# LuZWCHA/MLIC

Measured on AMD Instinct MI355X. Metric: images/sec (enc+dec) at 1920×1088 MLICPP_L, 1/2/4/8 GPU; bpp/PSNR Δ vs ref, higher is better.
Workload: dtype f32 (dense convs: f32 via split-fp16 MFMA, 3 terms); 1 GPU; config 2: MLICPP_L compress+decompress of 1920x1088 images (full rANS bitstreams, inputs resident in HBM); model=MLICPP_L, global_batch=32, per_gpu_images=32, weights=rate set(s) [1] of synthetic.RATE_LAMBDAS, parallelism=image-sharded x1 (no cross-GPU context), request_streams=4, schedule=each request stream runs its K steps back to back (no per-step join)

## Files before the change

mlic_amd/csrc/conv_x4.hip:

```cpp
#include "common.h"
#include "kernels.h"

#include <cstdio>
#include <type_traits>
#include <utility>
#include <vector>

namespace mlic {

typedef float floatx4 __attribute__((ext_vector_type(4)));
typedef _Float16 half8 __attribute__((ext_vector_type(8)));

namespace {
constexpr int X4T = 512;
constexpr int TR = 8, TC = 32;
constexpr int BN = TR * TC;
constexpr int ROWB = 128;
constexpr int ROWH = 64;

__device__ __forceinline__ int swz(int row) { return (row >> 1) & 7; }

__device__ __forceinline__ void glds16(const void* src, void* lds) {
  __builtin_amdgcn_global_load_lds((const __attribute__((address_space(1))) void*)src,
                                   (__attribute__((address_space(3))) void*)lds, 16, 0, 0);
}

__device__ __forceinline__ void glds16_asm(const void* src, const void* lds) {
  const uint32_t l = __builtin_amdgcn_readfirstlane(
      (uint32_t)reinterpret_cast<uintptr_t>((const __attribute__((address_space(3))) void*)lds));
  asm volatile("s_mov_b32 m0, %1\n\ts_nop 0\n\tglobal_load_lds_dwordx4 %0, off" : : "v"(src), "s"(l) : "m0");
}

__device__ __forceinline__ half8 lds_frag(const char* base, int row, int granule) {
  return *reinterpret_cast<const half8*>(base + row * ROWB + ((granule ^ swz(row)) << 4));
}
}

#ifndef MLIC_X4_ABL_RS
#define MLIC_X4_ABL_RS 0
#endif
#ifndef MLIC_X4_SPREAD
#define MLIC_X4_SPREAD 0
#endif
#ifndef MLIC_X4_STAGGER
#define MLIC_X4_STAGGER 0
#endif
template <int K, int BM, bool RS, bool HI, bool DIR = false, bool HALO = false>
__global__ __launch_bounds__(X4T) void conv_x4_kernel(ConvParams P, const _Float16* __restrict__ act,
                                                      const _Float16* __restrict__ wx, int nchunk, int H, int W,
                                                      int abl, int nsplit) {
  constexpr int KK = K * K;
  constexpr int WAVES_M = BM == 192 ? 4 : (BM == 96 || BM == 224) ? 2 : BM / 64, WAVES_N = 8 / WAVES_M;
  constexpr int WN = BN / WAVES_N;
  constexpr int TM = BM / (16 * WAVES_M), TN = WN / 16;
  constexpr int WR = 16 * TM;
  constexpr int A_BYTES = BM * ROWB, B_BYTES = BN * ROWB;
  constexpr int NAB = RS ? 2 : 3;
  constexpr int HR = TR + K - 1, HC = TC + K - 1, HLINES = HR * HC;
  constexpr int BSLOT = HALO ? HLINES * ROWB : B_BYTES;
  constexpr int B_OFF = NAB * A_BYTES, LDS = NAB * A_BYTES + 2 * BSLOT;
  constexpr int NA = A_BYTES / 1024 / 8;
  constexpr int NB = B_BYTES / 1024 / 8;
  static_assert(NA >= 1 && NB == 4 && LDS <= 160 * 1024, "x4 tile");
  static_assert(!HALO || (RS && !DIR && K > 1), "x4 halo: register-staged K x K only");
  __shared__ __attribute__((aligned(1024))) char sm[LDS];

  const int tid = threadIdx.x, lane = tid & 63, wave = tid >> 6;
  const int wm = wave / WAVES_N, wn = wave % WAVES_N;
  const int pad = K / 2;
  const int npix = P.Ho * P.Wo;
  const int S = K == 1 ? 1 : P.stride;
  const int Hp = (K == 1 ? H : P.H) + 2 * pad, Wp = (K == 1 ? W : P.W) + 2 * pad;
  const int ntx = (W + TC - 1) / TC;
  const int nct = gridDim.x, npt = gridDim.y, nblk = nct * npt;
  const int bid = blockIdx.y * nct + blockIdx.x;
  int logical = bid;
  if (nblk >= 16) {
    const int xcd = bid & 7, q = nblk >> 3, r = nblk & 7;
    logical = (xcd < r ? xcd * (q + 1) : r * (q + 1) + (xcd - r) * q) + (bid >> 3);
  }
  constexpr int XG = 4;
  int ct, pt;
  if (K == 1 && nct >= 2 * XG) {
    const int band = XG * npt, g = logical / band, first = g * XG, r = logical - g * band;
    const int gs = min(XG, nct - first);
    ct = first + r % gs;
    pt = r / gs;
  } else {
    ct = logical % nct;
    pt = logical / nct;
  }
  const int oy0 = (pt / ntx) * TR, ox0 = (pt % ntx) * TC;
  const int b = blockIdx.z % P.B, split = blockIdx.z / P.B;
  const int nsteps = nchunk * KK;
  const int s0 = HALO ? split * nchunk / nsplit * KK : split * nsteps / nsplit;
  const int s1 = HALO ? (split + 1) * nchunk / nsplit * KK : (split + 1) * nsteps / nsplit;
  if (nsplit > 1) P.out += (int64_t)split * P.B * P.out_bs;

  const int64_t plane = (int64_t)Hp * Wp * ROWH;
  const _Float16* bsrc[NB];
#pragma unroll
  for (int i = 0; i < NB; ++i) {
    const int n = (wave * NB + i) * 8 + (lane >> 3);
    const int oy = min(oy0 + n / TC, H - 1), ox = min(ox0 + n % TC, W - 1);
    const int G = (lane & 7) ^ swz(n);
    bsrc[i] = act + (int64_t)b * nchunk * plane + ((int64_t)oy * S * Wp + ox * S) * ROWH + G * 8;
  }
  const _Float16* asrc = wx + ((int64_t)ct * nsteps * BM) * ROWH + (wave * NA) * 512 + lane * 8;

  auto glds_one = [&](int g, int sb, int sa, int abuf) {
    if (g < NB) {
      const int cc = sb / KK, tap = sb - cc * KK;
      const int ky = tap / K, kx = tap - ky * K;
      const int64_t d = cc * plane + ((int64_t)ky * Wp + kx) * ROWH;
      glds16_asm(bsrc[g] + d, sm + B_OFF + (sb & 1) * B_BYTES + (wave * NB + g) * 1024);
    } else {
      const int i = g - NB;
      glds16_asm(asrc + (int64_t)sa * BM * ROWH + i * 512, sm + abuf * A_BYTES + (wave * NA + i) * 1024);
    }
  };
  constexpr int NG = NA + NB;

  floatx4 acc[TM][TN];
#pragma unroll
  for (int i = 0; i < TM; ++i)
#pragma unroll
    for (int j = 0; j < TN; ++j) acc[i][j] = floatx4{0.f, 0.f, 0.f, 0.f};

  const int G = lane >> 4, l16 = lane & 15;
  if constexpr (RS) {
    typedef unsigned int u32x4 __attribute__((ext_vector_type(4)));
    constexpr int NPA = A_BYTES / 1024, NAR = (NPA + 7) / 8;
    constexpr bool SPREAD = MLIC_X4_SPREAD && !DIR && !HALO && !HI;
    const _Float16* asrc_rs = wx + ((int64_t)ct * nsteps * BM) * ROWH + wave * 512 + lane * 8;
    u32x4 rb[(DIR || HALO) ? 1 : NB], ra[NAR];
    constexpr int NPH = (HLINES * 8 + X4T - 1) / X4T;
    static_assert(!HALO || NPH + 1 <= KK, "x4 halo: the next chunk's pieces must land within the chunk");
    u32x4 hb;
    const _Float16* himg = act + (int64_t)b * nchunk * plane;
    auto hsrc = [&](int q) __attribute__((always_inline)) {
      const int id = q * X4T + tid, line = min(id >> 3, HLINES - 1);
      const int hr = line / HC, hc = line - hr * HC;
      const int y = min(oy0 + hr, Hp - 1), x = min(ox0 + hc, Wp - 1);
      return ((int64_t)y * Wp + x) * ROWH + (id & 7) * 8;
    };
    auto hdst = [&](int q, int slot) __attribute__((always_inline)) {
      const int id = q * X4T + tid, line = id >> 3;
      return sm + B_OFF + slot * BSLOT + line * ROWB + (((id & 7) ^ swz(line)) << 4);
    };
    auto hvalid = [&](int q) __attribute__((always_inline)) { return q * X4T + tid < HLINES * 8; };
    float rv[DIR ? 16 : 1];
    const int dn = (wave & 3) * 64 + lane, dch = (wave >> 2) * 16;
    const int dp = min(oy0 * TC + dn, npix - 1);
    uint32_t dmax = 0;
    auto gload = [&](int st) __attribute__((always_inline)) {
      const int cc = st / KK, tap = st - cc * KK;
      const int ky = tap / K, kx = tap - ky * K;
      if constexpr (DIR) {
        const int ch0 = cc * 32 + dch;
        const float* sp = P.seg[0].p;
        int64_t sbs = P.seg[0].bs;
        int c0 = 0, cend = 0;
#pragma unroll
        for (int k = 1; k < MAXSEG; ++k) {
          cend += P.seg[k - 1].C;
          uint64_t pk = (uint64_t)P.seg[k].p, bk = (uint64_t)P.seg[k].bs;
          asm("" : "+s"(pk), "+s"(bk));
          if (k < P.nseg && ch0 >= cend) {
            sp = (const float*)pk;
            sbs = (int64_t)bk;
            c0 = cend;
          }
        }
        typedef const __attribute__((address_space(1))) float gfloat;
        gfloat* src = (gfloat*)(sp + (int64_t)b * sbs + (int64_t)(ch0 - c0) * npix) + dp;
        const int nval = P.Cin - ch0;
        if (nval >= 16) {
#pragma unroll
          for (int j = 0; j < 16; ++j) rv[j] = src[(int64_t)j * npix];
        } else {
#pragma unroll
          for (int j = 0; j < 16; ++j) rv[j] = j < nval ? src[(int64_t)j * npix] : 0.0f;
        }
      } else if constexpr (!HALO) {
        const int64_t d = cc * plane + ((int64_t)ky * Wp + kx) * ROWH;
#pragma unroll
        for (int i = 0; i < NB; ++i) rb[i] = *reinterpret_cast<const u32x4*>(bsrc[i] + d);
      }
#pragma unroll
      for (int i = 0; i < NAR; ++i)
        if (NPA % 8 == 0 || wave + 8 * i < NPA)
          ra[i] = *reinterpret_cast<const u32x4*>(asrc_rs + (int64_t)st * BM * ROWH + i * 8 * 512);
    };
    auto lstore = [&](int st) __attribute__((always_inline)) {
      if constexpr (DIR) {
        typedef float float2v __attribute__((ext_vector_type(2)));
        typedef _Float16 half2v __attribute__((ext_vector_type(2)));
        char* row = sm + B_OFF + (st & 1) * B_BYTES + dn * ROWB;
        const int sw = swz(dn), g0 = dch / 8;
#pragma unroll
        for (int q = 0; q < 2; ++q) {
          half8 h, l;
#pragma unroll
          for (int j = 0; j < 8; j += 2) {
            const float2v v = {rv[8 * q + j], rv[8 * q + j + 1]};
            const half2v hv = __builtin_convertvector(v, half2v);
            const half2v lv = __builtin_convertvector(v - __builtin_convertvector(hv, float2v), half2v);
            h[j] = hv[0];
            h[j + 1] = hv[1];
            l[j] = lv[0];
            l[j + 1] = lv[1];
            dmax = max(dmax, max(__float_as_uint(v[0]) & 0x7fffffffu, __float_as_uint(v[1]) & 0x7fffffffu));
          }
          *reinterpret_cast<half8*>(row + (((g0 + q) ^ sw) << 4)) = h;
          *reinterpret_cast<half8*>(row + (((g0 + q + 4) ^ sw) << 4)) = l;
        }
      } else if constexpr (!HALO) {
#pragma unroll
        for (int i = 0; i < NB; ++i)
          *reinterpret_cast<u32x4*>(sm + B_OFF + (st & 1) * B_BYTES + (wave * NB + i) * 1024 + lane * 16) = rb[i];
      }
#pragma unroll
      for (int i = 0; i < NAR; ++i)
        if (NPA % 8 == 0 || wave + 8 * i < NPA)
          *reinterpret_cast<u32x4*>(sm + (st & 1) * A_BYTES + (wave + 8 * i) * 1024 + lane * 16) = ra[i];
    };
    constexpr int NPC = NB + NAR;
    auto gload_piece = [&](int st, int p) __attribute__((always_inline)) {
      if (p < NB) {
        const int cc = st / KK, tap = st - cc * KK;
        const int ky = tap / K, kx = tap - ky * K;
        const int64_t d = cc * plane + ((int64_t)ky * Wp + kx) * ROWH;
        rb[p] = *reinterpret_cast<const u32x4*>(bsrc[p] + d);
      } else {
        const int i = p - NB;
        if (NPA % 8 == 0 || wave + 8 * i < NPA)
          ra[i] = *reinterpret_cast<const u32x4*>(asrc_rs + (int64_t)st * BM * ROWH + i * 8 * 512);
      }
    };
    auto lstore_piece = [&](int st, int p) __attribute__((always_inline)) {
      if (p < NB) {
        *reinterpret_cast<u32x4*>(sm + B_OFF + (st & 1) * B_BYTES + (wave * NB + p) * 1024 + lane * 16) = rb[p];
      } else {
        const int i = p - NB;
        if (NPA % 8 == 0 || wave + 8 * i < NPA)
          *reinterpret_cast<u32x4*>(sm + (st & 1) * A_BYTES + (wave + 8 * i) * 1024 + lane * 16) = ra[i];
      }
    };
    auto mfma_step = [&](int s, auto jh_c, auto&& hook) {
      constexpr int JH = decltype(jh_c)::value;
      const char* As = sm + (s & 1) * A_BYTES;
      const char* Bs;
      int tapoff = 0;
      if constexpr (HALO) {
        const int cc = s / KK, tap = s - cc * KK, ky = tap / K;
        Bs = sm + B_OFF + (cc & 1) * BSLOT;
        tapoff = ky * HC + (tap - ky * K);
      } else {
        Bs = sm + B_OFF + (s & 1) * B_BYTES;
      }
      auto brow = [&](int n) __attribute__((always_inline)) {
        return HALO ? (n / TC) * HC + (n % TC) + tapoff : n;
      };
      half8 ah[TM], al[TM];
#pragma unroll
      for (int i = 0; i < TM; ++i) {
        const int row = wm * WR + i * 16 + l16;
        ah[i] = lds_frag(As, row, G);
        al[i] = lds_frag(As, row, G + 4);
      }
      half8 bh[2], bl[2];
      bh[0] = lds_frag(Bs, brow(wn * WN + l16), G);
      bl[0] = lds_frag(Bs, brow(wn * WN + l16), G + 4);
#pragma unroll
      for (int j = 0; j < TN; ++j) {
        if (j + 1 < TN) {
          const int n = brow(wn * WN + (j + 1) * 16 + l16);
          bh[(j + 1) & 1] = lds_frag(Bs, n, G);
          bl[(j + 1) & 1] = lds_frag(Bs, n, G + 4);
        }
        if constexpr ((MLIC_X4_ABL_RS & 2) != 0) {
          asm volatile("" :: "v"(bh[j & 1]), "v"(bl[j & 1]));
          if (j == 0)
#pragma unroll
            for (int i = 0; i < TM; ++i) asm volatile("" :: "v"(ah[i]), "v"(al[i]));
        } else if constexpr (HI) {
#pragma unroll
          for (int i = 0; i < TM; ++i)
            acc[i][j] = __builtin_amdgcn_mfma_f32_16x16x32_f16(ah[i], bh[j & 1], acc[i][j], 0, 0, 0);
#pragma unroll
          for (int i = 0; i < TM; ++i)
            acc[i][j] = __builtin_amdgcn_mfma_f32_16x16x32_f16(al[i], bl[j & 1], acc[i][j], 0, 0, 0);
        } else {
#pragma unroll
          for (int i = 0; i < TM; ++i)
            acc[i][j] = __builtin_amdgcn_mfma_f32_16x16x32_f16(al[i], bh[j & 1], acc[i][j], 0, 0, 0);
#pragma unroll
          for (int i = 0; i < TM; ++i)
            acc[i][j] = __builtin_amdgcn_mfma_f32_16x16x32_f16(ah[i], bl[j & 1], acc[i][j], 0, 0, 0);
#pragma unroll
          for (int i = 0; i < TM; ++i)
            acc[i][j] = __builtin_amdgcn_mfma_f32_16x16x32_f16(ah[i], bh[j & 1], acc[i][j], 0, 0, 0);
        }
        if constexpr (SPREAD) {
          if ((j + 1) * NPC / TN > j * NPC / TN) {
            __builtin_amdgcn_sched_barrier(0);
            hook(j);
            __builtin_amdgcn_sched_barrier(0);
          }
        } else if (j == JH) {
          __builtin_amdgcn_sched_barrier(0);
          hook(j);
          __builtin_amdgcn_sched_barrier(0);
        }
      }
    };
    if (HALO && s0 < s1) {
      const int c0 = s0 / KK;
#pragma unroll
      for (int q = 0; q < NPH; ++q)
        if (hvalid(q)) {
          const u32x4 v = *reinterpret_cast<const u32x4*>(himg + c0 * plane + hsrc(q));
          *reinterpret_cast<u32x4*>(hdst(q, c0 & 1)) = v;
        }
    }
    if (s0 < s1) {
      gload(s0);
      lstore(s0);
    }
    if (s0 + 1 < s1) gload(s0 + 1);
    auto kloop = [&](auto jh_c) __attribute__((always_inline)) {
    for (int s = s0; s < s1; ++s) {
      asm volatile("s_waitcnt lgkmcnt(0)" ::: "memory");
      if constexpr ((MLIC_X4_ABL_RS & 4) == 0) __builtin_amdgcn_s_barrier();
      asm volatile("" ::: "memory");
      auto staging = [&](int j) __attribute__((always_inline)) {
        if constexpr ((MLIC_X4_ABL_RS & 1) != 0) return;
        if constexpr (SPREAD) {
#pragma unroll
          for (int p = 0; p < NPC; ++p)
            if (p >= j * NPC / TN && p < (j + 1) * NPC / TN) {
              if (s + 1 < s1) lstore_piece(s + 1, p);
              if (s + 2 < s1) gload_piece(s + 2, p);
            }
          return;
        }
        if (s + 1 < s1) lstore(s + 1);
        if constexpr (HALO) {
          const int cc = s / KK, j = s - cc * KK;
          if ((cc + 1) * KK < s1) {
            if (j >= 1 && j <= NPH && hvalid(j - 1)) *reinterpret_cast<u32x4*>(hdst(j - 1, (cc + 1) & 1)) = hb;
            if (j < NPH && hvalid(j)) hb = *reinterpret_cast<const u32x4*>(himg + (cc + 1) * plane + hsrc(j));
          }
        }
        if (s + 2 < s1) gload(s + 2);
      };
#ifdef MLIC_X4_STAGING_FIRST
      staging(0);
      mfma_step(s, jh_c, [](int) {});
#else
      mfma_step(s, jh_c, staging);
#endif
    }
    };
    if constexpr (MLIC_X4_STAGGER && K > 1) {
      if (__builtin_amdgcn_readfirstlane(wave) & 4) kloop(std::integral_constant<int, TN / 2>{});
      else kloop(std::integral_constant<int, 0>{});
    } else {
      kloop(std::integral_constant<int, 0>{});
    }
    if constexpr (DIR) range_report(P.rflag, f16_unsafe(__uint_as_float(dmax)));
  } else {
  static_assert(!HI, "the reduced-precision form runs on the register-staged path");
#pragma unroll
  for (int g = NB; g < NG; ++g) glds_one(g, 0, 0, 0);
#pragma unroll
  for (int g = 0; g < NB; ++g) glds_one(g, 0, 0, 0);
#pragma unroll
  for (int g = NB; g < NG; ++g) glds_one(g, 0, min(1, nsteps - 1), 1);
  int acur = 0;
  for (int s = 0; s < ((abl & 8) ? 0 : nsteps); ++s) {
    static_assert(NA == 1 || NA == 2 || NA == 4, "vmcnt immediate");
    if constexpr (NA == 4) asm volatile("s_waitcnt vmcnt(4)" ::: "memory");
    else if constexpr (NA == 2) asm volatile("s_waitcnt vmcnt(2)" ::: "memory");
    else asm volatile("s_waitcnt vmcnt(1)" ::: "memory");
    __builtin_amdgcn_s_barrier();
    asm volatile("" ::: "memory");
    const int sb = min(s + 1, nsteps - 1), sa = min(s + 2, nsteps - 1);
    const int anext = acur == 0 ? 2 : acur - 1;
    const char* As = sm + acur * A_BYTES;
    const char* Bs = sm + B_OFF + (s & 1) * B_BYTES;
    acur = acur == 2 ? 0 : acur + 1;
    half8 ah[TM], al[TM];
#pragma unroll
    for (int i = 0; i < TM; ++i) {
      const int row = wm * WR + i * 16 + l16;
      ah[i] = lds_frag(As, row, G);
      al[i] = lds_frag(As, row, G + 4);
    }
    half8 bh[2], bl[2];
    bh[0] = lds_frag(Bs, wn * WN + l16, G);
    bl[0] = lds_frag(Bs, wn * WN + l16, G + 4);
#pragma unroll
    for (int j = 0; j < TN; ++j) {
      if (!(abl & 1)) {
#pragma unroll
        for (int g = j * NG / TN; g < (j + 1) * NG / TN; ++g) glds_one(g, sb, sa, anext);
      }
      __builtin_amdgcn_sched_barrier(0);
      if (j + 1 < TN) {
        const int n = wn * WN + (j + 1) * 16 + l16;
        bh[(j + 1) & 1] = lds_frag(Bs, n, G);
        bl[(j + 1) & 1] = lds_frag(Bs, n, G + 4);
      }
      if (abl & 2) {
        asm volatile("" :: "v"(bh[j & 1]), "v"(bl[j & 1]));
        continue;
      }
#pragma unroll
      for (int i = 0; i < TM; ++i)
        acc[i][j] = __builtin_amdgcn_mfma_f32_16x16x32_f16(al[i], bh[j & 1], acc[i][j], 0, 0, 0);
#pragma unroll
      for (int i = 0; i < TM; ++i)
        acc[i][j] = __builtin_amdgcn_mfma_f32_16x16x32_f16(ah[i], bl[j & 1], acc[i][j], 0, 0, 0);
#pragma unroll
      for (int i = 0; i < TM; ++i)
        acc[i][j] = __builtin_amdgcn_mfma_f32_16x16x32_f16(ah[i], bh[j & 1], acc[i][j], 0, 0, 0);
    }

  }
  }

  constexpr int EP = WN + 4;
  asm volatile("s_waitcnt vmcnt(0)" ::: "memory");
  __syncthreads();
  if (abl & 4) {
#pragma unroll
    for (int i = 0; i < TM; ++i)
#pragma unroll
      for (int j = 0; j < TN; ++j) asm volatile("" :: "v"(acc[i][j]));
    return;
  }
  float* ep = reinterpret_cast<float*>(sm) + wave * 16 * EP;
  const int co_w = ct * BM + wm * WR;
  const bool shuf = (P.epi & EPI_SHUFFLE) != 0;
  const bool vec = conv_vec_ok(P) && !(shuf && (P.epi & (EPI_GDN | EPI_IGDN | EPI_MASK_ANCHOR | EPI_MASK_NONANCHOR)));
#pragma unroll
  for (int i = 0; i < TM; ++i) {
#pragma unroll
    for (int j = 0; j < TN; ++j)
#pragma unroll
      for (int e = 0; e < 4; ++e) ep[(4 * G + e) * EP + j * 16 + l16] = acc[i][j][e];
#pragma unroll 1
    for (int k = 0; k < WN / 16; ++k) {
      const int idx = k * 64 + lane;
      int r0, n;
      float4 v;
      if (!shuf) {
        r0 = idx / (WN / 4);
        n = 4 * (idx % (WN / 4));
        v = *reinterpret_cast<const float4*>(ep + r0 * EP + n);
      } else {
        const int combo = idx / (WN / 2);
        r0 = 4 * (combo >> 1) + 2 * (combo & 1);
        n = 2 * (idx % (WN / 2));
        const float2 c0 = *reinterpret_cast<const float2*>(ep + r0 * EP + n);
        const float2 c1 = *reinterpret_cast<const float2*>(ep + (r0 + 1) * EP + n);
        v = make_float4(c0.x, c1.x, c0.y, c1.y);
      }
      const int nn = wn * WN + n;
      const int oy = oy0 + nn / TC, ox = ox0 + nn % TC;
      const int co = co_w + i * 16 + r0;
      const int p = oy * W + ox;
      if (oy >= H || ox >= W || p >= npix) continue;
      if (!shuf) {
        if (vec && co < P.Cout && ox + 3 < W && p + 3 < npix) {
          conv_store4(P, b, co, p, v);
        } else if (co < P.Cout) {
          const float vs[4] = {v.x, v.y, v.z, v.w};
#pragma unroll
          for (int e = 0; e < 4; ++e)
            if (ox + e < W && p + e < npix) conv_store(P, b, co, p + e, vs[e]);
        }
      } else {
        if (vec && co + 1 < P.Cout && ox + 1 < W) {
          conv_store_shuf4(P, b, co, p, v);
        } else {
          if (co < P.Cout) conv_store(P, b, co, p, v.x);
          if (co + 1 < P.Cout) conv_store(P, b, co + 1, p, v.y);
          if (ox + 1 < W) {
            if (co < P.Cout) conv_store(P, b, co, p + 1, v.z);
            if (co + 1 < P.Cout) conv_store(P, b, co + 1, p + 1, v.w);
          }
        }
      }
    }
  }
}

struct X4Pack {
  Seg seg[MAXSEG];
  int nseg, Cin, H, W, pad, nchunk, square, npix;
  int relu;
  int hi;
  _Float16* dst;
  int* rflag;
};

__global__ __launch_bounds__(256) void x4_pack_act_kernel(X4Pack Q) {
  const int Hp = Q.H + 2 * Q.pad, Wp = Q.W + 2 * Q.pad;
  const int pos = blockIdx.x * 64 + (threadIdx.x & 63);
  const int g = threadIdx.x >> 6;
  const int cc = blockIdx.y, b = blockIdx.z;
  const int y = pos / Wp - Q.pad, x = pos % Wp - Q.pad;
  const bool inb = pos < Hp * Wp && y >= 0 && y < Q.H && x >= 0 && x < Q.W && y * Q.W + x < Q.npix;
  const int64_t HW = Q.npix;
  bool bad = false;
  auto load8 = [&](int ch0, float (&v)[8]) {
    int s = 0, c0 = 0;
    while (s + 1 < Q.nseg && ch0 >= c0 + Q.seg[s].C) { c0 += Q.seg[s].C; ++s; }
    const Seg sg = Q.seg[s];
    const float* src = sg.p + (int64_t)b * sg.bs + (int64_t)(ch0 - c0) * HW + (int64_t)y * Q.W + x;
#pragma unroll
    for (int j = 0; j < 8; ++j) {
      const bool ok = inb && ch0 + j < Q.Cin && ch0 - c0 + j < sg.C;
      v[j] = ok ? src[(int64_t)j * HW] : 0.0f;
      if (Q.square) v[j] *= v[j];
      if (Q.relu) v[j] = v[j] < 0.0f ? 0.0f : v[j];
      bad |= f16_unsafe(v[j]);
    }
  };
  half8 h, l;
  float v[8];
  if (Q.hi) {
    load8(cc * 64 + 8 * g, v);
#pragma unroll
    for (int j = 0; j < 8; ++j) h[j] = (_Float16)v[j];
    load8(cc * 64 + 32 + 8 * g, v);
#pragma unroll
    for (int j = 0; j < 8; ++j) l[j] = (_Float16)v[j];
  } else {
    load8(cc * 32 + 8 * g, v);
#pragma unroll
    for (int j = 0; j < 8; ++j) {
      const _Float16 hv = (_Float16)v[j];
      h[j] = hv;
      l[j] = (_Float16)(v[j] - (float)hv);
    }
  }
  constexpr int SP = ROWH + 8;
  __shared__ __attribute__((aligned(16))) _Float16 stg[64 * SP];
  const int lane = threadIdx.x & 63;
  *reinterpret_cast<half8*>(stg + lane * SP + 8 * g) = h;
  *reinterpret_cast<half8*>(stg + lane * SP + 32 + 8 * g) = l;
  __syncthreads();
  const int nlines = min(64, Hp * Wp - (int)blockIdx.x * 64);
  _Float16* d = Q.dst + (((int64_t)b * Q.nchunk + cc) * Hp * Wp + (int64_t)blockIdx.x * 64) * ROWH;
#pragma unroll
  for (int k = 0; k < 2; ++k) {
    const int q = k * 256 + threadIdx.x;
    if (q / 8 < nlines)
      *reinterpret_cast<half8*>(d + q * 8) = *reinterpret_cast<const half8*>(stg + (q / 8) * SP + (q % 8) * 8);
  }
  range_report(Q.rflag, bad);
}

struct LinAttPack {
  const float* Q;
  int64_t q_bs;
  const float* ctx;
  int heads, H, W, pad, nchunk, qmask;
  _Float16* dst;
  int* rflag;
};

template <int HD>
__global__ __launch_bounds__(256) void linatt_pack_kernel(LinAttPack A) {
  constexpr int HPC = 32 / HD;
  __shared__ __attribute__((aligned(16))) float cs[HPC * HD * HD];
  const int Hp = A.H + 2 * A.pad, Wp = A.W + 2 * A.pad, HW = A.H * A.W;
  const int cc = blockIdx.y, b = blockIdx.z;
  const float* cb = A.ctx + ((int64_t)b * A.heads + cc * HPC) * HD * HD;
  for (int i = threadIdx.x; i < HPC * HD * HD; i += 256) cs[i] = cb[i];
  __syncthreads();
  const int pos = blockIdx.x * 64 + (threadIdx.x & 63);
  const int g = threadIdx.x >> 6;
  const int y = pos / Wp - A.pad, x = pos % Wp - A.pad;
  const bool inb = pos < Hp * Wp && y >= 0 && y < A.H && x >= 0 && x < A.W;
  const int hl = (8 * g) / HD, d0 = (8 * g) % HD;
  float a[8];
#pragma unroll
  for (int j = 0; j < 8; ++j) a[j] = 0.0f;
  if (inb && !(A.qmask && is_anchor(y, x))) {
    float q[HD];
    query_softmax<HD>(A.Q + (int64_t)b * A.q_bs + (int64_t)(cc * HPC + hl) * HD * HW + (int64_t)y * A.W + x, HW, q);
    const float* w = cs + hl * HD * HD + d0;
#pragma unroll
    for (int c = 0; c < HD; ++c) {
      const float4 w0 = *reinterpret_cast<const float4*>(w + c * HD), w1 = *reinterpret_cast<const float4*>(w + c * HD + 4);
      a[0] = fmaf(w0.x, q[c], a[0]);
      a[1] = fmaf(w0.y, q[c], a[1]);
      a[2] = fmaf(w0.z, q[c], a[2]);
      a[3] = fmaf(w0.w, q[c], a[3]);
      a[4] = fmaf(w1.x, q[c], a[4]);
      a[5] = fmaf(w1.y, q[c], a[5]);
      a[6] = fmaf(w1.z, q[c], a[6]);
      a[7] = fmaf(w1.w, q[c], a[7]);
    }
  }
  bool bad = false;
  half8 h, l;
#pragma unroll
  for (int j = 0; j < 8; ++j) {
    const _Float16 hv = (_Float16)a[j];
    h[j] = hv;
    l[j] = (_Float16)(a[j] - (float)hv);
    bad |= f16_unsafe(a[j]);
  }
  constexpr int SP = ROWH + 8;
  __shared__ __attribute__((aligned(16))) _Float16 stg[64 * SP];
  const int lane = threadIdx.x & 63;
  *reinterpret_cast<half8*>(stg + lane * SP + 8 * g) = h;
  *reinterpret_cast<half8*>(stg + lane * SP + 32 + 8 * g) = l;
  __syncthreads();
  const int nlines = min(64, Hp * Wp - (int)blockIdx.x * 64);
  _Float16* d = A.dst + (((int64_t)b * A.nchunk + cc) * Hp * Wp + (int64_t)blockIdx.x * 64) * ROWH;
#pragma unroll
  for (int k = 0; k < 2; ++k) {
    const int q = k * 256 + threadIdx.x;
    if (q / 8 < nlines)
      *reinterpret_cast<half8*>(d + q * 8) = *reinterpret_cast<const half8*>(stg + (q / 8) * SP + (q % 8) * 8);
  }
  range_report(A.rflag, bad);
}

void linatt_pack(const float* Q, int64_t q_bs, const float* ctx, int heads, int hd, int qmask, const ConvParams& P,
                 _Float16* dst, hipStream_t st) {
  MLIC_CHECK((hd == 16 || hd == 32) && P.Cin == heads * hd && P.Cin % 32 == 0 && P.K > 1 && P.stride == 1,
             "linatt_pack: shape");
  LinAttPack A{};
  A.Q = Q;
  A.q_bs = q_bs;
  A.ctx = ctx;
  A.heads = heads;
  A.H = P.H;
  A.W = P.W;
  A.pad = P.K / 2;
  A.nchunk = P.Cin / 32;
  A.qmask = qmask;
  A.dst = dst;
  A.rflag = P.rflag;
  const int npos = (A.H + 2 * A.pad) * (A.W + 2 * A.pad);
  const dim3 grid((npos + 63) / 64, A.nchunk, P.B);
  if (hd == 16) hipLaunchKernelGGL(linatt_pack_kernel<16>, grid, dim3(256), 0, st, A);
  else hipLaunchKernelGGL(linatt_pack_kernel<32>, grid, dim3(256), 0, st, A);
  HIP_OK(hipGetLastError());
}

__global__ void x4_pack_weights_kernel(const _Float16* __restrict__ wh, const _Float16* __restrict__ wl,
                                       _Float16* __restrict__ dst, int Cout, int KK, int cin_pad, int BM,
                                       int64_t n, int hi) {
  const int64_t i = (int64_t)blockIdx.x * blockDim.x + threadIdx.x;
  if (i >= n) return;
  const int e = (int)(i % ROWH);
  const int row = (int)((i / ROWH) % BM);
  const int64_t ts = i / ((int64_t)ROWH * BM);
  const int nchunk = hi ? (cin_pad + 63) / 64 : cin_pad / 32, nsteps = nchunk * KK;
  const int step = (int)(ts % nsteps), ct = (int)(ts / nsteps);
  const int cc = step / KK, tap = step - cc * KK;
  const int Gp = e >> 3, G = Gp ^ ((row >> 1) & 7);
  const int k = (G & 3) * 8 + (e & 7);
  const int co = ct * BM + row;
  _Float16 v = (_Float16)0.0f;
  if (co < Cout) {
    const int ch = hi ? cc * 64 + (G >> 2) * 32 + k : cc * 32 + k;
    const int64_t off = ((int64_t)co * KK + tap) * cin_pad + ch;
    if (hi) v = ch < cin_pad ? wh[off] : (_Float16)0.0f;
    else v = G < 4 ? wh[off] : wl[off];
  }
  dst[i] = v;
}

int x4_bm(int Cout) {
  static const std::vector<std::pair<int, int>> force = [] {
    std::vector<std::pair<int, int>> v;
    for (const char* q = opt_str(OPT_X4_BM_FOR); q && *q;) {
      int c = 0, m = 0, n = 0;
      if (std::sscanf(q, "%d:%d%n", &c, &m, &n) != 2) break;
      if (m == 64 || m == 96 || m == 128 || m == 192 || m == 224 || m == 256) v.emplace_back(c, m);
      q += n;
      if (*q == ',') ++q;
    }
    return v;
  }();
  for (const auto& f : force)
    if (f.first == Cout) return f.second;
  if (Cout <= 64) return 64;
  if (Cout == 1280) return 128;
  if (opt(OPT_X4_BM96) && Cout > 64 && Cout <= 96) return 96;
  if (Cout > 128 && Cout <= 192) return 192;
  if (opt(OPT_X4_BM224) && Cout > 192 && Cout <= 224) return 224;
  const int w256 = (Cout + 255) / 256 * 256 - Cout, w128 = (Cout + 127) / 128 * 128 - Cout;
  return (Cout >= 192 && 8 * (w256 - w128) <= Cout) ? 256 : 128;
}

int x4_nchunk(int cin_pad, bool hi) { return hi ? (cin_pad + 63) / 64 : cin_pad / 32; }

int64_t x4_weight_halves(int Cout, int KK, int cin_pad, bool hi) {
  const int bm = x4_bm(Cout);
  return (int64_t)((Cout + bm - 1) / bm) * bm * KK * x4_nchunk(cin_pad, hi) * ROWH;
}

void x4_pack_weights(const _Float16* wh, const _Float16* wl, int Cout, int KK, int cin_pad, _Float16* dst,
                     hipStream_t st, bool hi) {
  const int64_t n = x4_weight_halves(Cout, KK, cin_pad, hi);
  hipLaunchKernelGGL(x4_pack_weights_kernel, dim3((unsigned)((n + 255) / 256)), dim3(256), 0, st, wh, wl, dst, Cout,
                     KK, cin_pad, x4_bm(Cout), n, hi ? 1 : 0);
  HIP_OK(hipGetLastError());
}
static void x4_grid(const ConvParams& P, int& H, int& W) {
  H = P.K == 1 ? (P.H * P.W + TC - 1) / TC : P.H;
  W = P.K == 1 ? TC : P.W;
}
static void x4_tgrid(const ConvParams& P, int& H, int& W) {
  H = P.K == 1 ? (P.H * P.W + TC - 1) / TC : P.Ho;
  W = P.K == 1 ? TC : P.Wo;
}

int64_t x4_act_halves(const ConvParams& P, int cin_pad, bool hi) {
  const int pad = P.K / 2;
  int H, W;
  x4_grid(P, H, W);
  return (int64_t)P.B * x4_nchunk(cin_pad, hi) * (H + 2 * pad) * (W + 2 * pad) * ROWH;
}

bool conv_x4_ok(const ConvParams& P, int cin_pad) {
  if (!(P.K == 1 || P.K == 3 || P.K == 5) || P.pad != P.K / 2) return false;
  if (!(P.stride == 1 || (P.stride == 2 && P.K == 3))) return false;
  if (P.Ho != (P.H - 1) / P.stride + 1 || P.Wo != (P.W - 1) / P.stride + 1) return false;
  if (cin_pad % 32 != 0 || cin_pad < P.Cin || P.Cout < 32) return false;
  for (int s = 0; s + 1 < P.nseg; ++s)
    if (P.seg[s].C % 16 != 0) return false;
  return true;
}

void x4_pack_act(const ConvParams& P, int cin_pad, _Float16* dst, hipStream_t st, bool hi) {
  X4Pack Q{};
  for (int s = 0; s < P.nseg; ++s) Q.seg[s] = P.seg[s];
  Q.nseg = P.nseg;
  Q.Cin = P.Cin;
  x4_grid(P, Q.H, Q.W);
  Q.npix = P.H * P.W;
  Q.pad = P.K / 2;
  Q.nchunk = x4_nchunk(cin_pad, hi);
  Q.hi = hi ? 1 : 0;
  Q.square = (P.epi & EPI_SQUARE_IN) ? 1 : 0;
  Q.relu = (P.epi & EPI_RELU_IN) ? 1 : 0;
  Q.dst = dst;
  Q.rflag = P.rflag;
  const int npos = (Q.H + 2 * Q.pad) * (Q.W + 2 * Q.pad);
  hipLaunchKernelGGL(x4_pack_act_kernel, dim3((npos + 63) / 64, Q.nchunk, P.B), dim3(256), 0, st, Q);
  HIP_OK(hipGetLastError());
}

__global__ __launch_bounds__(256) void x4_split_reduce_kernel(ConvParams P, const float* __restrict__ part,
                                                              int nsplit) {
  const int HWo = P.Ho * P.Wo;
  const int64_t n = (int64_t)P.B * P.Cout * HWo;
  const int64_t i = (int64_t)blockIdx.x * 256 + threadIdx.x;
  if (i >= n) return;
  const int p = (int)(i % HWo);
  const int64_t r = i / HWo;
  const int co = (int)(r % P.Cout), b = (int)(r / P.Cout);
  float v = part[i];
  for (int k = 1; k < nsplit; ++k) v += part[(int64_t)k * n + i];
  conv_store(P, b, co, p, v);
}

static bool x4_rs() { return opt(OPT_X4_RS) != 0; }

template <int K, int BM>
constexpr bool x4_halo_fits() {
  constexpr int a = 2 * BM * ROWB, h = 2 * (TR + K - 1) * (TC + K - 1) * ROWB;
  return K > 1 && a + h <= 160 * 1024;
}
static bool x4_halo(const ConvParams& P, bool hi) {
  const int setting = opt(OPT_X4_HALO);
  if (setting == 0 || P.K == 1 || P.stride != 1) return false;
  if (P.K == 3 && setting != 2) return false;
  const int bm = x4_bm(P.Cout);
  return 2 * bm * ROWB + 2 * (TR + P.K - 1) * (TC + P.K - 1) * ROWB <= 160 * 1024;
}

bool x4_direct_ok(const ConvParams& P, bool hi) {
  return opt(OPT_X4_DIRECT) && P.K == 1 && !hi && !(P.epi & (EPI_SQUARE_IN | EPI_RELU_IN)) && x4_rs();
}

template <int K, int BM>
static void launch_x4(const ConvParams& P, const _Float16* act, const _Float16* wx, int nchunk, hipStream_t st,
                      int nsplit, bool hi) {
  int H, W;
  x4_tgrid(P, H, W);
  const int ntx = (W + TC - 1) / TC, nty = (H + TR - 1) / TR;
  dim3 grid((P.Cout + BM - 1) / BM, ntx * nty, P.B * nsplit);
  const int abl = opt(OPT_X4_ABL);
  if (K == 1 && !act)
    hipLaunchKernelGGL((conv_x4_kernel<K, BM, true, false, K == 1>), grid, dim3(X4T), 0, st, P, act, wx, nchunk, H, W,
                       abl, nsplit);
  else if (hi && x4_halo(P, hi)) {
    if constexpr (x4_halo_fits<K, BM>())
      hipLaunchKernelGGL((conv_x4_kernel<K, BM, true, true, false, true>), grid, dim3(X4T), 0, st, P, act, wx, nchunk,
                         H, W, abl, nsplit);
  } else if (hi)
    hipLaunchKernelGGL((conv_x4_kernel<K, BM, true, true>), grid, dim3(X4T), 0, st, P, act, wx, nchunk, H, W, abl,
                       nsplit);
  else if (x4_rs() && x4_halo(P, hi)) {
    if constexpr (x4_halo_fits<K, BM>())
      hipLaunchKernelGGL((conv_x4_kernel<K, BM, true, false, false, true>), grid, dim3(X4T), 0, st, P, act, wx, nchunk,
                         H, W, abl, nsplit);
  } else if (x4_rs())
    hipLaunchKernelGGL((conv_x4_kernel<K, BM, true, false>), grid, dim3(X4T), 0, st, P, act, wx, nchunk, H, W, abl,
                       nsplit);
  else if constexpr (BM != 192 && BM != 96 && BM != 224)
    hipLaunchKernelGGL((conv_x4_kernel<K, BM, false, false>), grid, dim3(X4T), 0, st, P, act, wx, nchunk, H, W, abl, 1);
  else
    hipLaunchKernelGGL((conv_x4_kernel<K, BM, true, false>), grid, dim3(X4T), 0, st, P, act, wx, nchunk, H, W, abl,
                       nsplit);
  HIP_OK(hipGetLastError());
}

int x4_splitk(const ConvParams& P, int cin_pad, bool hi) {
  if (!opt(OPT_X4_SPLITK) || !x4_rs() || P.K == 1) return 1;
  int H, W;
  x4_tgrid(P, H, W);
  const int tiles = ((P.Cout + x4_bm(P.Cout) - 1) / x4_bm(P.Cout)) * ((W + TC - 1) / TC) * ((H + TR - 1) / TR);
  const int nsteps = x4_nchunk(cin_pad, hi) * P.K * P.K;
  if (tiles > 48 || nsteps < 48) return 1;
  const int s = std::min(4, nsteps / 24);
  return x4_halo(P, hi) ? std::max(1, std::min(s, x4_nchunk(cin_pad, hi))) : s;
}

int64_t x4_part_bytes(const ConvParams& P, int cin_pad, bool hi) {
  const int s = x4_splitk(P, cin_pad, hi);
  return s > 1 ? (int64_t)s * P.B * P.Cout * P.Ho * P.Wo * 4 : 0;
}

void conv_x4_forward(const ConvParams& P, const _Float16* act, const _Float16* wx, int cin_pad, hipStream_t st,
                     float* part, bool hi) {
  MLIC_CHECK(conv_x4_ok(P, cin_pad) && wx && (act || x4_direct_ok(P, hi)), "conv_x4: unsupported shape");
  ConvParams Q = P;
  if (act) Q.epi &= ~(EPI_SQUARE_IN | EPI_RELU_IN);
  const int nchunk = x4_nchunk(cin_pad, hi);
  const int bm = x4_bm(P.Cout);
  const int nsplit = part ? x4_splitk(P, cin_pad, hi) : 1;
  ConvParams R = Q;
  if (nsplit > 1) {
    R.epi = EPI_NONE;
    R.bias = nullptr;
    R.wexp = 0;
    R.aux = nullptr;
    R.res = nullptr;
    R.out = part;
    R.out_cs = (int64_t)P.Ho * P.Wo;
    R.out_bs = (int64_t)P.Cout * R.out_cs;
  }
#define MLIC_X4_BM(K)                                                  \
  (bm == 256 ? launch_x4<K, 256>(R, act, wx, nchunk, st, nsplit, hi)       \
   : bm == 192 ? launch_x4<K, 192>(R, act, wx, nchunk, st, nsplit, hi)     \
   : bm == 96 ? launch_x4<K, 96>(R, act, wx, nchunk, st, nsplit, hi)       \
   : bm == 224 ? launch_x4<K, 224>(R, act, wx, nchunk, st, nsplit, hi)     \
   : bm == 128 ? launch_x4<K, 128>(R, act, wx, nchunk, st, nsplit, hi)     \
               : launch_x4<K, 64>(R, act, wx, nchunk, st, nsplit, hi))
  switch (P.K) {
    case 1: MLIC_X4_BM(1); break;
    case 3: MLIC_X4_BM(3); break;
    default: MLIC_X4_BM(5); break;
  }
#undef MLIC_X4_BM
  if (nsplit > 1) {
    const int64_t n = (int64_t)P.B * P.Cout * P.Ho * P.Wo;
    hipLaunchKernelGGL(x4_split_reduce_kernel, dim3((unsigned)((n + 255) / 256)), dim3(256), 0, st, Q,
                       (const float*)part, nsplit);
    HIP_OK(hipGetLastError());
  }
}

}
```

Before: 113.1 images/sec.

## Pad and skew halo LDS rows to avoid bank conflicts; enable halo for 3x3

The halo B-tile in LDS now uses a padded 144-byte row pitch with a skewed granule placement instead of the 128-byte XOR-swizzled rows, and B fragments are read through a precomputed per-lane base. Because halo rows are addressed at arbitrary tap offsets, the XOR swizzle no longer lines up, and padding is meant to remove the LDS bank conflicts this causes. The launch rule also turns on the halo path for 3x3 convs under the default setting, which reuses the activation halo across taps instead of restaging each tap. The cost is more LDS per block, which may exclude some tile sizes or lower occupancy.

```diff
diff --git a/mlic_amd/csrc/conv_x4.hip b/mlic_amd/csrc/conv_x4.hip
--- a/mlic_amd/csrc/conv_x4.hip
+++ b/mlic_amd/csrc/conv_x4.hip
@@ -17,6 +17,27 @@
 constexpr int BN = TR * TC;
 constexpr int ROWB = 128;
 constexpr int ROWH = 64;
+
+#ifndef MLIC_X4_HALO_PITCH
+#define MLIC_X4_HALO_PITCH 144
+#endif
+#ifndef MLIC_X4_HALO_SKEW
+#define MLIC_X4_HALO_SKEW (MLIC_X4_HALO_PITCH == 144)
+#endif
+constexpr int HPITCH = MLIC_X4_HALO_PITCH;
+constexpr bool HPAD = HPITCH != ROWB;
+constexpr bool HSKEW = MLIC_X4_HALO_SKEW;
+static_assert(HPITCH == ROWB || (HPITCH >= ROWB + 16 && HPITCH % 16 == 0), "x4 halo pitch");
+static_assert(!HSKEW || HPITCH == 144, "x4 halo skew: 9-granule rows");
+__host__ __device__ constexpr int hgran(int g) {
+  return (HSKEW ? ((g >> 1) & 1) + (g >> 2) * 4 + (g & 1) * 16 : g) * 16;
+}
+constexpr int HLO = hgran(4) - hgran(0);
+static_assert(hgran(5) - hgran(1) == HLO && hgran(6) - hgran(2) == HLO && hgran(7) - hgran(3) == HLO, "x4 halo lo offset");
+constexpr int HTAIL = (HPAD && hgran(7) + 16 > HPITCH) ? hgran(7) + 16 - HPITCH : 0;
+constexpr int x4_halo_lds(int K, int bm) {
+  return 2 * bm * ROWB + 2 * (TR + K - 1) * (TC + K - 1) * HPITCH + HTAIL;
+}
 
 __device__ __forceinline__ int swz(int row) { return (row >> 1) & 7; }
 
@@ -57,8 +78,9 @@
   constexpr int A_BYTES = BM * ROWB, B_BYTES = BN * ROWB;
   constexpr int NAB = RS ? 2 : 3;
   constexpr int HR = TR + K - 1, HC = TC + K - 1, HLINES = HR * HC;
-  constexpr int BSLOT = HALO ? HLINES * ROWB : B_BYTES;
-  constexpr int B_OFF = NAB * A_BYTES, LDS = NAB * A_BYTES + 2 * BSLOT;
+  constexpr int BSLOT = HALO ? HLINES * HPITCH : B_BYTES;
+  constexpr int B_OFF = NAB * A_BYTES, LDS = NAB * A_BYTES + 2 * BSLOT + (HALO ? HTAIL : 0);
+  static_assert(!HALO || LDS == x4_halo_lds(K, BM), "x4 halo: the launch rule's footprint");
   constexpr int NA = A_BYTES / 1024 / 8;
   constexpr int NB = B_BYTES / 1024 / 8;
   static_assert(NA >= 1 && NB == 4 && LDS <= 160 * 1024, "x4 tile");
@@ -146,7 +168,8 @@
     };
     auto hdst = [&](int q, int slot) __attribute__((always_inline)) {
       const int id = q * X4T + tid, line = id >> 3;
-      return sm + B_OFF + slot * BSLOT + line * ROWB + (((id & 7) ^ swz(line)) << 4);
+      if constexpr (HPAD) return sm + B_OFF + slot * BSLOT + line * HPITCH + hgran(id & 7);
+      else return sm + B_OFF + slot * BSLOT + line * ROWB + (((id & 7) ^ swz(line)) << 4);
     };
     auto hvalid = [&](int q) __attribute__((always_inline)) { return q * X4T + tid < HLINES * 8; };
     float rv[DIR ? 16 : 1];
@@ -247,6 +270,8 @@
           *reinterpret_cast<u32x4*>(sm + (st & 1) * A_BYTES + (wave + 8 * i) * 1024 + lane * 16) = ra[i];
       }
     };
+    static_assert(WN % TC == 0, "x4: a wave's pixels are whole tile rows");
+    const int hlane = (wn * (WN / TC) * HC + l16) * HPITCH + hgran(G);
     auto mfma_step = [&](int s, auto jh_c, auto&& hook) {
       constexpr int JH = decltype(jh_c)::value;
       const char* As = sm + (s & 1) * A_BYTES;
@@ -262,6 +287,11 @@
       auto brow = [&](int n) __attribute__((always_inline)) {
         return HALO ? (n / TC) * HC + (n % TC) + tapoff : n;
       };
+      constexpr bool HP = HALO && HPAD;
+      const char* Bp = HP ? Bs + hlane + tapoff * HPITCH : nullptr;
+      auto hfrag = [&](int j, int lo) __attribute__((always_inline)) {
+        return *reinterpret_cast<const half8*>(Bp + ((j * 16 / TC) * HC + j * 16 % TC) * HPITCH + lo * HLO);
+      };
       half8 ah[TM], al[TM];
 #pragma unroll
       for (int i = 0; i < TM; ++i) {
@@ -270,14 +300,24 @@
         al[i] = lds_frag(As, row, G + 4);
       }
       half8 bh[2], bl[2];
-      bh[0] = lds_frag(Bs, brow(wn * WN + l16), G);
-      bl[0] = lds_frag(Bs, brow(wn * WN + l16), G + 4);
+      if constexpr (HP) {
+        bh[0] = hfrag(0, 0);
+        bl[0] = hfrag(0, 1);
+      } else {
+        bh[0] = lds_frag(Bs, brow(wn * WN + l16), G);
+        bl[0] = lds_frag(Bs, brow(wn * WN + l16), G + 4);
+      }
 #pragma unroll
       for (int j = 0; j < TN; ++j) {
         if (j + 1 < TN) {
-          const int n = brow(wn * WN + (j + 1) * 16 + l16);
-          bh[(j + 1) & 1] = lds_frag(Bs, n, G);
-          bl[(j + 1) & 1] = lds_frag(Bs, n, G + 4);
+          if constexpr (HP) {
+            bh[(j + 1) & 1] = hfrag(j + 1, 0);
+            bl[(j + 1) & 1] = hfrag(j + 1, 1);
+          } else {
+            const int n = brow(wn * WN + (j + 1) * 16 + l16);
+            bh[(j + 1) & 1] = lds_frag(Bs, n, G);
+            bl[(j + 1) & 1] = lds_frag(Bs, n, G + 4);
+          }
         }
         if constexpr ((MLIC_X4_ABL_RS & 2) != 0) {
           asm volatile("" :: "v"(bh[j & 1]), "v"(bl[j & 1]));
@@ -781,15 +821,14 @@
 
 template <int K, int BM>
 constexpr bool x4_halo_fits() {
-  constexpr int a = 2 * BM * ROWB, h = 2 * (TR + K - 1) * (TC + K - 1) * ROWB;
-  return K > 1 && a + h <= 160 * 1024;
+  return K > 1 && x4_halo_lds(K, BM) <= 160 * 1024;
 }
 static bool x4_halo(const ConvParams& P, bool hi) {
   const int setting = opt(OPT_X4_HALO);
   if (setting == 0 || P.K == 1 || P.stride != 1) return false;
-  if (P.K == 3 && setting != 2) return false;
+  if (P.K == 3 && setting == 5) return false;
   const int bm = x4_bm(P.Cout);
-  return 2 * bm * ROWB + 2 * (TR + P.K - 1) * (TC + P.K - 1) * ROWB <= 160 * 1024;
+  return x4_halo_lds(P.K, bm) <= 160 * 1024;
 }
 
 bool x4_direct_ok(const ConvParams& P, bool hi) {
```

New measurement: 115.7 images/sec, median of 6. 1.02x the previous value.
